# SamArgt/AudioSourceSep

Hardware: AMD Instinct MI355X
Metric: Glow fwd+logdet passes/sec on 64×64×1 mel tiles (K=32,L=3), 1→8 MI355X (higher is better)
Workload: dtype f16x3

## Files before the change

### audiosourcesep_amd/csrc/glowk_co.h

```cpp
#pragma once
#include "glowk_kernels.h"

constexpr int CO_PX = 128;
constexpr int CO_PSTR = 132;

template <int KIN, int MOUT, int NF, int MODE>
struct RingC {
  static constexpr int MODE7 = net_dir<MODE>;
  using S = RingS<KIN, MOUT, NF, MODE7, 2>;
  static constexpr bool FUSE = (MODE & NET_FUSE) != 0;
  static constexpr bool SAVE = MODE7 == NET_FWD_SAVE, BWD = MODE7 == NET_BWD;
  static constexpr bool MERGE = S::NMT <= 3;
  static constexpr bool M0LAST = S::NMT % 3 == 2;
  static constexpr bool STORE = (MODE & NET_STORE) != 0;
  static constexpr int MODEX = net_dir<MODE> | (MODE & NET_STORE);
  static constexpr int NFH = S::NFH, NRB = S::NRB, NMT = S::NMT, KS = S::KS;
  static constexpr int UNITP = S::MAINP / 2;
  static constexpr int UNIT4 = S::MAIN4 / 2;
  static constexpr int PPW = UNITP / 4;
  static constexpr int NG = NFH / 2;
  static constexpr int K1PW = (S::K1P + 3) / 4;
  static constexpr int EPN = BWD ? 0 : S::EPN;
  static constexpr int MASKN = BWD ? 2 * 4 * NF * 64 : 0;
  static constexpr size_t LDS_BYTES = (size_t)3 * UNIT4 * 16 + (size_t)2 * S::K14 * 16 + (size_t)EPN * 4 + (size_t)MASKN * 2 +
// ... 67 lines not shown
    acc2[o1][0] = __builtin_amdgcn_mfma_f32_16x16x32_f16(af[3], bh[0], acc2[o1][0], 0, 0, 0);
    acc2[o1][1] = __builtin_amdgcn_mfma_f32_16x16x32_f16(af[3], bh[1], acc2[o1][1], 0, 0, 0);
    if (MODE7 != NET_FWD2) {
      acc2[o0][0] = __builtin_amdgcn_mfma_f32_16x16x32_f16(af[0], bl[0], acc2[o0][0], 0, 0, 0);
      acc2[o0][1] = __builtin_amdgcn_mfma_f32_16x16x32_f16(af[0], bl[1], acc2[o0][1], 0, 0, 0);
      acc2[o1][0] = __builtin_amdgcn_mfma_f32_16x16x32_f16(af[2], bl[0], acc2[o1][0], 0, 0, 0);
      acc2[o1][1] = __builtin_amdgcn_mfma_f32_16x16x32_f16(af[2], bl[1], acc2[o1][1], 0, 0, 0);
    }
    acc2[o0][0] = __builtin_amdgcn_mfma_f32_16x16x32_f16(af[0], bh[0], acc2[o0][0], 0, 0, 0);
    acc2[o0][1] = __builtin_amdgcn_mfma_f32_16x16x32_f16(af[0], bh[1], acc2[o0][1], 0, 0, 0);
    acc2[o1][0] = __builtin_amdgcn_mfma_f32_16x16x32_f16(af[2], bh[0], acc2[o1][0], 0, 0, 0);
    acc2[o1][1] = __builtin_amdgcn_mfma_f32_16x16x32_f16(af[2], bh[1], acc2[o1][1], 0, 0, 0);
    __builtin_amdgcn_sched_barrier(0);
  }
}

template <int KIN, int MOUT, int NF, int MODE, int PASS, bool SOLO, int Z>
__device__ __forceinline__ void co_Z(const NetArgs& a, const H3Ctx& hc, const CoCtx& c, const float* epl, float* pl,
                                     f32x4 (&acc2)[(RingC<KIN, MOUT, NF, MODE>::NRB)][2], f32x4 (&acc3)[(RingC<KIN, MOUT, NF, MODE>::NMT)][2], h8 (&bh)[2],
                                     h8 (&bl)[2], const int (&q)[2], const bool (&qok)[2], int lane, int kq,
                                     f32x4 (&keep)[(RingC<KIN, MOUT, NF, MODE>::NMT)][2]) {
  using G = RingC<KIN, MOUT, NF, MODE>;
  constexpr int NFH = G::NFH, NMT = G::NMT, M3 = MOUT, MODE7 = G::MODE7;
  constexpr bool NEXT = !SOLO && PASS == 0;
  constexpr bool LAST = !SOLO && PASS == 1;
  if constexpr (NMT == 3) {
    if constexpr (Z == 0) stage4<G::UNITP, 70>(G::out_unit(c.img, PASS, 2), c.m1, c.w4, c.voff);
    if constexpr (Z == 1 && NEXT) stage4<G::UNITP, 71>(G::out_unit(c.img, PASS + 1, 0), c.d, c.w4, c.voff);
    if constexpr (Z == 2 && NEXT) stage4<G::UNITP, 72>(G::main_unit(c.img, PASS + 1, 0, 0), c.m0, c.w4, c.voff);
  } else if constexpr (NMT == 2) {
    if constexpr (Z == 0 && NEXT) stage4<G::UNITP, 75>(G::main_unit(c.img, PASS + 1, 0, 1), c.m1, c.w4, c.voff);
    if constexpr (Z == 1 && NEXT) stage4<G::UNITP, 76>(G::out_unit(c.img, PASS + 1, 0), c.d, c.w4, c.voff);
  } else {
    static_assert(NMT == 5, "conv3 units");
    if constexpr (Z == 0) stage4<G::UNITP, 80>(G::out_unit(c.img, PASS, 2), c.m1, c.w4, c.voff);
    if constexpr (Z == 1) stage4<G::UNITP, 81>(G::out_unit(c.img, PASS, 3), c.d, c.w4, c.voff);
    if constexpr (Z == 2) stage4<G::UNITP, 82>(G::out_unit(c.img, PASS, 4), c.m0, c.w4, c.voff);
    if constexpr (Z == 3 && NEXT) stage4<G::UNITP, 83>(G::main_unit(c.img, PASS + 1, 0, 1), c.m1, c.w4, c.voff);
    if constexpr (Z == 4 && NEXT) stage4<G::UNITP, 84>(G::out_unit(c.img, PASS + 1, 0), c.d, c.w4, c.voff);
  }
  const float4* slot = Z % 3 == 0 ? c.d : Z % 3 == 1 ? c.m0 : c.m1;
  const h8* buf = reinterpret_cast<const h8*>(slot) + lane;
  const float* pb = epl + NF * 32;
#pragma unroll
  for (int tp = 0; tp < NFH; ++tp) {
    const int t = Z * NFH + tp;
    const int fo = t / NMT, ml = t % NMT;
    if (ml == 0) {
      unsigned mask = 0, bits = 0;
      if (G::BWD) mask = hc.mkl[((size_t)(threadIdx.x >> 6) * NF + PASS * NFH + fo) * 64 + lane];
      if constexpr (G::STORE)
        bits = h3s_act_pair<MODE7, true>(acc2[2 * fo][0], acc2[2 * fo + 1][0], acc2[2 * fo][1], acc2[2 * fo + 1][1], a.sc2, mask, bh, bl,
                                         uniform_fptr(a.st2 + (size_t)(PASS * NFH + fo) * 32 * a.Q), ((unsigned)(4 * kq) * (unsigned)a.Q + (unsigned)q[0]) * 4u,
                                         (unsigned)a.Q * 4u);
      else {
#pragma unroll
        for (int hf = 0; hf < 2; ++hf) bits |= h3s_act<MODE7, false>(acc2[2 * fo][hf], acc2[2 * fo + 1][hf], a.sc2, mask >> (8 * hf), bh[hf], bl[hf]) << (8 * hf);
      }
      if (G::SAVE && hc.wok) a.mask2[(hc.wblk * NF + PASS * NFH + fo) * 64 + lane] = (unsigned short)bits;
    }
    if (fo == 0) {
#pragma unroll
      for (int r = 0; r < 4; ++r) { acc3[ml][0][r] = 0.0f; acc3[ml][1][r] = 0.0f; }
    }
    const h8 ah = buf[(tp * 2 + 0) * 64], al = buf[(tp * 2 + 1) * 64];
    acc3[ml][0] = mfma3s<MODE7 == NET_FWD2>(ah, al, bh[0], bl[0], acc3[ml][0]);
    acc3[ml][1] = mfma3s<MODE7 == NET_FWD2>(ah, al, bh[1], bl[1], acc3[ml][1]);
    if (fo == NFH - 1) {
#pragma unroll
      for (int hf = 0; hf < 2; ++hf)
#pragma unroll
        for (int r = 0; r < 4; ++r) {
          const int m = ml * 16 + 4 * kq + r;
          const float part = G::BWD ? acc3[ml][hf][r] * (a.sc3 * hc.ub[hf]) : PASS == 0 ? fmaf(acc3[ml][hf][r], a.sc3, pb[m]) : acc3[ml][hf][r] * a.sc3;
          if constexpr (NEXT && G::MERGE) { keep[ml][hf][r] = part; continue; }
          const float val = (LAST && G::MERGE) ? part + keep[ml][hf][r] : part;
          if constexpr (G::FUSE) {
            if (m < M3) pl[m * CO_PSTR + (int)(threadIdx.x >> 6) * 32 + 16 * hf + (lane & 15)] = val;
          } else {
            float* Pp = a.P + ((SOLO || !G::MERGE) ? (size_t)PASS * a.pstride : (size_t)0);
            if (m < M3 && qok[hf]) Pp[(size_t)m * a.Q + q[hf]] = val;
          }
        }
    }
  }
  constexpr bool ISSUED = NMT == 3 ? (Z == 0 || NEXT) : NMT == 2 ? (Z <= 1 && NEXT) : (Z <= 2 || NEXT);
  if constexpr (Z + 1 < NMT) {
    if constexpr (G::STORE) {
      constexpr int after = (ISSUED ? G::PPW : 0) + G::z_st(Z) + ((NMT == 3 && Z == 1) ? G::z_st(0) : 0);
      co_end<(after < 63 ? after : 63)>();
    } else if constexpr (G::SAVE) co_end<0>();
    else co_end<(ISSUED ? G::PPW : 0)>();
  } else co_bar();
}

template <int KIN, int MOUT, int NF, int MODE, int PASS, bool SOLO>
__device__ __forceinline__ void co_pass(const NetArgs& a, const H3Ctx& hc, const CoCtx& c, const float* epl, float* pl,
                                        const h8 (&xh)[(RingC<KIN, MOUT, NF, MODE>::KS)][2], const h8 (&xl)[(RingC<KIN, MOUT, NF, MODE>::KS)][2],
                                        const int (&q)[2], const bool (&qok)[2], int lane, int kq, f32x4 (&keep)[(RingC<KIN, MOUT, NF, MODE>::NMT)][2]) {
  using G = RingC<KIN, MOUT, NF, MODE>;
  using S = typename G::S;
  constexpr int NRB = G::NRB, NFH = G::NFH, MODE7 = G::MODE7;
  constexpr int f2base = PASS * NFH * 32;
  constexpr bool SECOND = !SOLO && PASS == 1;
  f32x4 acc2[NRB][2];
#pragma unroll
  for (int ob = 0; ob < NRB; ++ob)
#pragma unroll
    for (int r = 0; r < 4; ++r) {
      const float b = G::BWD ? 0.0f : epl[f2base + ob * 16 + 4 * kq + r];
      acc2[ob][0][r] = b;
      acc2[ob][1][r] = b;
    }
  const bool st = G::SAVE && PASS == 0 && hc.wok;
  constexpr int XST = PASS == 0 ? G::XST : 0;
  h8 bh[2], bl[2];
#pragma nounroll
  for (int i0 = 0; i0 < NF; i0 += 2) {
    if (i0 > 0 || (SECOND && !G::M0LAST)) stage4<G::UNITP, 73>(G::main_unit(c.img, PASS, i0, 1), c.m1, c.w4, c.voff);
    if constexpr (SECOND && G::M0LAST) {
      if (i0 == 0) stage4<G::UNITP, 77>(G::main_unit(c.img, PASS, 0, 0), c.m0, c.w4, c.voff);
    }
    h3s_X<KIN, MOUT, NF, G::MODEX, 2, 0, PASS, G::STORE>(a, hc, i0, xh, xl, lane, bh, bl);
    if (SECOND && G::M0LAST && i0 == 0) co_end<0>();
    else co_end_st<G::PPW + XST>(st);
    co_Y<NFH, MODE7, 0, 1, S::K1P>(c.m0, bh, bl, acc2, lane, hc.k1img + (size_t)((i0 + 2) % NF) * S::K14, hc.k1s0, c.w4, c.voff);
    co_end_st<G::K1PW + XST>(st);
    co_Y<NFH, MODE7, 1, 2, S::K1P>(c.m1, bh, bl, acc2, lane, G::main_unit(c.img, PASS, i0 + 1, 0), c.m0, c.w4, c.voff);
    co_bar();
    stage4<G::UNITP, 74>(G::main_unit(c.img, PASS, i0 + 1, 1), c.m1, c.w4, c.voff);
    h3s_X<KIN, MOUT, NF, G::MODEX, 2, 1, PASS, G::STORE>(a, hc, i0 + 1, xh, xl, lane, bh, bl);
    co_end_st<G::PPW + XST>(st);
    co_Y<NFH, MODE7, 0, 3, S::K1P>(c.m0, bh, bl, acc2, lane, hc.k1img + (size_t)((i0 + 3) % NF) * S::K14, hc.k1s1, c.w4, c.voff);
    co_end_st<G::K1PW + XST>(st);
    co_Y<NFH, MODE7, 1, 4, S::K1P>(c.m1, bh, bl, acc2, lane, i0 + 2 < NF ? G::main_unit(c.img, PASS, i0 + 2, 0) : G::out_unit(c.img, PASS, 1), c.m0,
                                   c.w4, c.voff);
    co_bar();
  }
  f32x4 acc3[G::NMT][2];
  co_Z<KIN, MOUT, NF, MODE, PASS, SOLO, 0>(a, hc, c, epl, pl, acc2, acc3, bh, bl, q, qok, lane, kq, keep);
  co_Z<KIN, MOUT, NF, MODE, PASS, SOLO, 1>(a, hc, c, epl, pl, acc2, acc3, bh, bl, q, qok, lane, kq, keep);
  if constexpr (G::NMT >= 3) co_Z<KIN, MOUT, NF, MODE, PASS, SOLO, 2>(a, hc, c, epl, pl, acc2, acc3, bh, bl, q, qok, lane, kq, keep);
  if constexpr (G::NMT >= 4) co_Z<KIN, MOUT, NF, MODE, PASS, SOLO, 3>(a, hc, c, epl, pl, acc2, acc3, bh, bl, q, qok, lane, kq, keep);
  if constexpr (G::NMT >= 5) co_Z<KIN, MOUT, NF, MODE, PASS, SOLO, 4>(a, hc, c, epl, pl, acc2, acc3, bh, bl, q, qok, lane, kq, keep);
}

struct CoCtxDB {
  float4 *s0, *s1, *s2, *s3;
  const float4* img;
  int w4;
  unsigned voff;
};

template <int NFH, int MODE7, int TAG, int K1P>
__device__ __forceinline__ void co_Ydb(const float4* sa, const float4* sb, const h8 (&bh)[2], const h8 (&bl)[2], f32x4 (&acc2)[2 * NFH][2], int lane,
                                       const float4* srca, float4* dsta, const float4* srcb, float4* dstb, const float4* k1src, float4* k1dst,
                                       int w4, unsigned voff) {
  const h8* bufa = reinterpret_cast<const h8*>(sa) + lane;
  const h8* bufb = reinterpret_cast<const h8*>(sb) + lane;
  const char* uba = uniform_ptr(srca);
  const char* ubb = uniform_ptr(srcb);
  constexpr int NG = NFH / 2;
  h8 A[2][4];
  auto load = [&](h8 (&d)[4], int g) {
    const h8* buf = g < NG ? bufa : bufb;
    const int gi = g % NG;
    d[0] = buf[((2 * gi) * 2 + 0) * 64];
    d[1] = buf[((2 * gi) * 2 + 1) * 64];
    d[2] = buf[((2 * gi + 1) * 2 + 0) * 64];
    d[3] = buf[((2 * gi + 1) * 2 + 1) * 64];
  };
  load(A[0], 0);
#pragma unroll
  for (int g = 0; g < 2 * NG; ++g) {
    const int gi = g % NG;
    const int o0 = (g / NG) * NFH + 2 * gi, o1 = o0 + 1;
    if (g + 1 < 2 * NG) load(A[(g + 1) & 1], g + 1);
    const int piece = gi * 4 + w4;
    if (g < NG) glds16(reinterpret_cast<const float4*>(uba + (size_t)piece * 1024 + voff), dsta + piece * 64);
    else glds16(reinterpret_cast<const float4*>(ubb + (size_t)piece * 1024 + voff), dstb + piece * 64);
    asm volatile("; dma site %0" ::"n"(TAG * 16 + g));
    if (g == 0) stage4<K1P, TAG * 16 + 15>(k1src, k1dst, w4, voff);
    __builtin_amdgcn_sched_barrier(0);
    const h8 (&af)[4] = A[g & 1];
    acc2[o0][0] = __builtin_amdgcn_mfma_f32_16x16x32_f16(af[1], bh[0], acc2[o0][0], 0, 0, 0);
    acc2[o0][1] = __builtin_amdgcn_mfma_f32_16x16x32_f16(af[1], bh[1], acc2[o0][1], 0, 0, 0);
    acc2[o1][0] = __builtin_amdgcn_mfma_f32_16x16x32_f16(af[3], bh[0], acc2[o1][0], 0, 0, 0);
    acc2[o1][1] = __builtin_amdgcn_mfma_f32_16x16x32_f16(af[3], bh[1], acc2[o1][1], 0, 0, 0);
    if (MODE7 != NET_FWD2) {
      acc2[o0][0] = __builtin_amdgcn_mfma_f32_16x16x32_f16(af[0], bl[0], acc2[o0][0], 0, 0, 0);
      acc2[o0][1] = __builtin_amdgcn_mfma_f32_16x16x32_f16(af[0], bl[1], acc2[o0][1], 0, 0, 0);
      acc2[o1][0] = __builtin_amdgcn_mfma_f32_16x16x32_f16(af[2], bl[0], acc2[o1][0], 0, 0, 0);
      acc2[o1][1] = __builtin_amdgcn_mfma_f32_16x16x32_f16(af[2], bl[1], acc2[o1][1], 0, 0, 0);
    }
    acc2[o0][0] = __builtin_amdgcn_mfma_f32_16x16x32_f16(af[0], bh[0], acc2[o0][0], 0, 0, 0);
    acc2[o0][1] = __builtin_amdgcn_mfma_f32_16x16x32_f16(af[0], bh[1], acc2[o0][1], 0, 0, 0);
    acc2[o1][0] = __builtin_amdgcn_mfma_f32_16x16x32_f16(af[2], bh[0], acc2[o1][0], 0, 0, 0);
    acc2[o1][1] = __builtin_amdgcn_mfma_f32_16x16x32_f16(af[2], bh[1], acc2[o1][1], 0, 0, 0);
    __builtin_amdgcn_sched_barrier(0);
  }
}

template <int KIN, int MOUT, int NF, int MODE, int PASS, int Z>
__device__ __forceinline__ void co_Zdb(const NetArgs& a, const CoCtxDB& c, const float* epl, f32x4 (&acc2)[(RingC<KIN, MOUT, NF, MODE>::NRB)][2],
                                       f32x4 (&acc3)[3][2], h8 (&bh)[2], h8 (&bl)[2], int lane, int kq, f32x4 (&keep)[3][2]) {
  using G = RingC<KIN, MOUT, NF, MODE>;
  constexpr int NFH = G::NFH, NMT = G::NMT, M3 = MOUT, MODE7 = G::MODE7;
  static_assert(NMT == 3 && G::MERGE && G::FUSE, "the double-buffered ring: three conv3 units, merged passes, fused coupling");
  constexpr bool NEXT = PASS == 0;
  if constexpr (Z == 0) stage4<G::UNITP, 90>(G::out_unit(c.img, PASS, 2), c.s2, c.w4, c.voff);
  if constexpr (Z == 1 && NEXT) stage4<G::UNITP, 91>(G::main_unit(c.img, PASS + 1, 0, 0), c.s0, c.w4, c.voff);
  if constexpr (Z == 2 && NEXT) stage4<G::UNITP, 92>(G::main_unit(c.img, PASS + 1, 0, 1), c.s1, c.w4, c.voff);
  const float4* slot = Z == 0 ? c.s0 : Z == 1 ? c.s1 : c.s2;
  const h8* buf = reinterpret_cast<const h8*>(slot) + lane;
  const float* pb = epl + NF * 32;
#pragma unroll
  for (int tp = 0; tp < NFH; ++tp) {
    const int t = Z * NFH + tp;
    const int fo = t / NMT, ml = t % NMT;
    if (ml == 0) {
#pragma unroll
      for (int hf = 0; hf < 2; ++hf) h3s_act<MODE7, false>(acc2[2 * fo][hf], acc2[2 * fo + 1][hf], a.sc2, 0u, bh[hf], bl[hf]);
    }
    if (fo == 0) {
#pragma unroll
      for (int r = 0; r < 4; ++r) { acc3[ml][0][r] = 0.0f; acc3[ml][1][r] = 0.0f; }
    }
    const h8 ah = buf[(tp * 2 + 0) * 64], al = buf[(tp * 2 + 1) * 64];
    acc3[ml][0] = mfma3s<MODE7 == NET_FWD2>(ah, al, bh[0], bl[0], acc3[ml][0]);
    acc3[ml][1] = mfma3s<MODE7 == NET_FWD2>(ah, al, bh[1], bl[1], acc3[ml][1]);
    if (fo == NFH - 1) {
      float* pt = reinterpret_cast<float*>(ml == 0 ? c.s0 : ml == 1 ? c.s1 : c.s3);
#pragma unroll
      for (int hf = 0; hf < 2; ++hf)
#pragma unroll
        for (int r = 0; r < 4; ++r) {
          const int m = ml * 16 + 4 * kq + r;
          const float part = PASS == 0 ? fmaf(acc3[ml][hf][r], a.sc3, pb[m]) : acc3[ml][hf][r] * a.sc3;
          if constexpr (NEXT) { keep[ml][hf][r] = part; continue; }
          const float val = part + keep[ml][hf][r];
          if (m < M3) pt[(4 * kq + r) * CO_PSTR + (int)(threadIdx.x >> 6) * 32 + 16 * hf + (lane & 15)] = val;
        }
    }
  }
  if constexpr (Z == 0) co_bar();
  if constexpr (Z == 1) co_end<(NEXT ? G::PPW : 0)>();
  if constexpr (Z == 2 && NEXT) co_bar();
}

template <int KIN, int MOUT, int NF, int MODE, int PASS>
__device__ __forceinline__ void co_pass_db(const NetArgs& a, const H3Ctx& hc, const CoCtxDB& c, const float* epl,
                                           const h8 (&xh)[(RingC<KIN, MOUT, NF, MODE>::KS)][2], const h8 (&xl)[(RingC<KIN, MOUT, NF, MODE>::KS)][2],
                                           int lane, int kq, f32x4 (&keep)[3][2]) {
  using G = RingC<KIN, MOUT, NF, MODE>;
  using S = typename G::S;
  constexpr int NRB = G::NRB, NFH = G::NFH, MODE7 = G::MODE7;
  constexpr int f2base = PASS * NFH * 32;
  f32x4 acc2[NRB][2];
#pragma unroll
  for (int ob = 0; ob < NRB; ++ob)
#pragma unroll
    for (int r = 0; r < 4; ++r) {
      const float b = epl[f2base + ob * 16 + 4 * kq + r];
      acc2[ob][0][r] = b;
      acc2[ob][1][r] = b;
    }
  h8 bh[2], bl[2];
#pragma nounroll
  for (int i0 = 0; i0 < NF; i0 += 2) {
    h3s_X<KIN, MOUT, NF, G::MODEX, 2, 0, PASS, false>(a, hc, i0, xh, xl, lane, bh, bl);
    co_end<0>();
    co_Ydb<NFH, MODE7, 1, S::K1P>(c.s0, c.s1, bh, bl, acc2, lane, G::main_unit(c.img, PASS, i0 + 1, 0), c.s2, G::main_unit(c.img, PASS, i0 + 1, 1), c.s3,
                                  hc.k1img + (size_t)((i0 + 2) % NF) * S::K14, hc.k1s0, c.w4, c.voff);
    h3s_X<KIN, MOUT, NF, G::MODEX, 2, 1, PASS, false>(a, hc, i0 + 1, xh, xl, lane, bh, bl);
    co_end<0>();
    const bool more = i0 + 2 < NF;
    co_Ydb<NFH, MODE7, 2, S::K1P>(c.s2, c.s3, bh, bl, acc2, lane, more ? G::main_unit(c.img, PASS, i0 + 2, 0) : G::out_unit(c.img, PASS, 0), c.s0,
                                  more ? G::main_unit(c.img, PASS, i0 + 2, 1) : G::out_unit(c.img, PASS, 1), c.s1,
                                  hc.k1img + (size_t)((i0 + 3) % NF) * S::K14, hc.k1s1, c.w4, c.voff);
  }
  co_end<0>();
  f32x4 acc3[3][2];
  co_Zdb<KIN, MOUT, NF, MODE, PASS, 0>(a, c, epl, acc2, acc3, bh, bl, lane, kq, keep);
  co_Zdb<KIN, MOUT, NF, MODE, PASS, 1>(a, c, epl, acc2, acc3, bh, bl, lane, kq, keep);
  co_Zdb<KIN, MOUT, NF, MODE, PASS, 2>(a, c, epl, acc2, acc3, bh, bl, lane, kq, keep);
}

template <int KIN, int MOUT, int NF, int MODE, bool SPLIT, bool RING3 = false>
__global__ __launch_bounds__(256, 2) void k_net_h3c(NetArgs a) {
  using G = RingC<KIN, MOUT, NF, MODE>;
  using S = typename G::S;
  constexpr int KS = G::KS;
  constexpr int SGN = G::BWD ? -1 : 1;
  static_assert(G::FITS, "shape");
  static_assert(!(G::FUSE && SPLIT), "the fused coupling needs both passes in one workgroup");
  constexpr bool DB = G::DB && !SPLIT && !RING3;
  static_assert(!RING3 || G::DB, "RING3 names the three-slot form of an instance that has both");
  static_assert(!DB || 2 * G::LDS_BYTES_DB <= 160 * 1024, "two workgroups per CU");

  const int tid = threadIdx.x;
  CoCtx c;
  CoCtxDB cd;
  if constexpr (DB) {
    __shared__ __attribute__((aligned(1024))) float4 slotS0[G::DBSLOT4];
    __shared__ __attribute__((aligned(1024))) float4 slotS1[G::DBSLOT4];
    __shared__ __attribute__((aligned(1024))) float4 slotS2[G::DBSLOT4];
    __shared__ __attribute__((aligned(1024))) float4 slotS3[G::DBSLOT4];
    cd.s0 = slotS0; cd.s1 = slotS1; cd.s2 = slotS2; cd.s3 = slotS3;
  } else {
    __shared__ __attribute__((aligned(1024))) float4 slotM0[G::UNIT4];
    __shared__ __attribute__((aligned(1024))) float4 slotM1[G::UNIT4];
    __shared__ __attribute__((aligned(1024))) float4 slotD[G::UNIT4];
    c.m0 = slotM0; c.m1 = slotM1; c.d = slotD;
  }
  __shared__ __attribute__((aligned(1024))) float4 k1slot0[S::K14];
  __shared__ __attribute__((aligned(1024))) float4 k1slot1[S::K14];
  float* epl = nullptr;
  if constexpr (!G::BWD) { __shared__ float epl_arr[S::EPN]; epl = epl_arr; }
  unsigned short* mkl = nullptr;
  if constexpr (G::BWD) { __shared__ __attribute__((aligned(1024))) unsigned short mkl_arr[G::MASKN]; mkl = mkl_arr; }
  float* plds = nullptr;
  float4* vstash = nullptr;
  if constexpr (G::FUSE && !DB) { __shared__ float plds_arr[36 * CO_PSTR]; plds = plds_arr; }
  if constexpr (G::FUSE) { __shared__ float4 vstash_arr[CO_PX]; vstash = vstash_arr; }
  const int lane = tid & 63;
  const int wave = __builtin_amdgcn_readfirstlane(tid >> 6);
  const int n16 = lane & 15;
  const int kq = lane >> 4;
  const int qbase = ((int)blockIdx.x * 4 + wave) * 32;
  const int q[2] = {G::STORE ? qbase + 2 * n16 : qbase + n16, G::STORE ? qbase + 2 * n16 + 1 : qbase + 16 + n16};
  const bool qok[2] = {q[0] < a.Q, q[1] < a.Q};
  const int pass0 = SPLIT ? (int)blockIdx.y : 0;

  H3Ctx hc;
  hc.sA = hc.sB = hc.sD = nullptr; hc.k1s0 = k1slot0; hc.k1s1 = k1slot1;
  hc.k1img = a.RSp; hc.img = a.RSp; hc.mkl = mkl; hc.mk2off = 4 * NF * 64; hc.pl = plds;
  hc.wblk = (size_t)blockIdx.x * 4 + wave;
  hc.wok = (long)hc.wblk * 32 < a.Q;
  hc.w4 = wave; hc.voff = (unsigned)lane * 16u; hc.ub[0] = hc.ub[1] = 1.0f;
  c.img = a.RSp; c.w4 = wave; c.voff = (unsigned)lane * 16u;
  cd.img = a.RSp; cd.w4 = wave; cd.voff = (unsigned)lane * 16u;

  if constexpr (DB) {
    stage4<G::UNITP, 58>(G::main_unit(cd.img, 0, 0, 0), cd.s0, c.w4, c.voff);
    stage4<G::UNITP, 59>(G::main_unit(cd.img, 0, 0, 1), cd.s1, c.w4, c.voff);
  } else {
    stage4<G::UNITP, 60>(G::main_unit(c.img, pass0, 0, 0), c.m0, c.w4, c.voff);
    stage4<G::UNITP, 61>(G::main_unit(c.img, pass0, 0, 1), c.m1, c.w4, c.voff);
    stage4<G::UNITP, 62>(G::out_unit(c.img, pass0, 0), c.d, c.w4, c.voff);
  }
  stage4<S::K1P, 63>(hc.k1img, k1slot0, c.w4, c.voff);
  stage4<S::K1P, 64>(hc.k1img + S::K14, k1slot1, c.w4, c.voff);
  if constexpr (G::BWD) {
    stage4<NF / 2, 65>(reinterpret_cast<const float4*>(a.mask1 + (size_t)blockIdx.x * 4 * NF * 64), reinterpret_cast<float4*>(mkl), c.w4, c.voff);
    stage4<NF / 2, 66>(reinterpret_cast<const float4*>(a.mask2 + (size_t)blockIdx.x * 4 * NF * 64), reinterpret_cast<float4*>(mkl + 4 * NF * 64), c.w4, c.voff);
  }

  h8 xh[KS][2], xl[KS][2];
  float xmax = 0.0f;
  {
    const int hw = a.h * a.w;
#pragma unroll
    for (int hf = 0; hf < 2; ++hf) {
      const int qq = qok[hf] ? q[hf] : 0;
      const int rem = qq % hw;
      const int i = rem / a.w, j0 = rem % a.w;
      const float* base = a.vin + (long)qq * a.in_stride + a.in_off;
      if constexpr (G::BWD) {
        float v[KS][8];
        float pm = 0.0f;
#pragma unroll
        for (int s = 0; s < KS; ++s) {
          gather8<KIN, false, SGN>(base, i, j0, a.h, a.w, a.in_stride, qok[hf], 32 * s + 8 * kq, v[s]);
          pm = range8(pm, v[s]);
        }
        pm = nan_max(pm, __shfl_xor(pm, 16, 64));
        pm = nan_max(pm, __shfl_xor(pm, 32, 64));
        xmax = nan_max(xmax, pm);
        const float fac = G::STORE ? 1.0f : pixel_norm(pm, a.bnorm, hc.ub[hf]);
#pragma unroll
        for (int s = 0; s < KS; ++s) {
#pragma unroll
          for (int j = 0; j < 8; ++j) v[s][j] *= fac;
          split8(v[s], xh[s][hf], xl[s][hf]);
        }
      } else if constexpr (S::STK) {
        xmax = gather_stacked<KIN, SGN, G::MODE7 == NET_FWD2, KS, S::KSX>(base, i, j0, a.h, a.w, a.in_stride, qok[hf], kq, xh, xl, hf, xmax);
      } else {
#pragma unroll
        for (int s = 0; s < KS; ++s) {
          float v[8];
          gather8<KIN, true, SGN>(base, i, j0, a.h, a.w, a.in_stride, qok[hf], 32 * s + 8 * kq, v);
          xmax = range8(xmax, v);
          split8(v, xh[s][hf], xl[s][hf]);
        }
      }
    }
  }
  if constexpr (G::FUSE) {
    if (tid < CO_PX) {
      const int qv = (int)blockIdx.x * CO_PX + tid;
      vstash[tid] = qv < a.Q ? *reinterpret_cast<const float4*>(a.vin + (size_t)qv * 4) : float4{0.f, 0.f, 0.f, 0.f};
    }
  }
  if constexpr (!G::BWD)
    for (int i = tid; i < S::EPN; i += 256) epl[i] = a.eph[i];
  if (((G::BWD && !G::STORE) ? !(xmax <= 3.0e38f) : !(xmax <= a.xlim)) && a.flag) *a.flag = 1;
  if (a.xmax_out) range_probe(a.xmax_out, xmax);
  asm volatile("s_waitcnt vmcnt(0)" ::: "memory");
  __syncthreads();

  f32x4 keep[G::NMT][2];
  if constexpr (DB) {
    co_pass_db<KIN, MOUT, NF, MODE, 0>(a, hc, cd, epl, xh, xl, lane, kq, keep);
    co_pass_db<KIN, MOUT, NF, MODE, 1>(a, hc, cd, epl, xh, xl, lane, kq, keep);
    __syncthreads();
    fused_couple<CO_PX, CO_PSTR>(a, reinterpret_cast<const float*>(cd.s0), reinterpret_cast<const float*>(cd.s1), reinterpret_cast<const float*>(cd.s3), vstash, tid);
  } else if constexpr (SPLIT) {
    if (pass0 == 0) co_pass<KIN, MOUT, NF, MODE, 0, true>(a, hc, c, epl, plds, xh, xl, q, qok, lane, kq, keep);
    else co_pass<KIN, MOUT, NF, MODE, 1, true>(a, hc, c, epl, plds, xh, xl, q, qok, lane, kq, keep);
  } else {
    co_pass<KIN, MOUT, NF, MODE, 0, false>(a, hc, c, epl, plds, xh, xl, q, qok, lane, kq, keep);
    co_pass<KIN, MOUT, NF, MODE, 1, false>(a, hc, c, epl, plds, xh, xl, q, qok, lane, kq, keep);
  }
  if constexpr (G::FUSE && !DB) {
    __syncthreads();
    fused_couple<CO_PX, CO_PSTR>(a, plds, vstash, tid);
  }
}
```

### audiosourcesep_amd/csrc/glowk_kernels.h

```cpp
#pragma once
#include "glowk_act_scale.h"

#include <hip/hip_runtime.h>
#include <utility>
#include <stdint.h>

typedef float f32x16 __attribute__((ext_vector_type(16)));

#define GLOWK_GPTR(p) ((const __attribute__((address_space(1))) void*)(p))
#define GLOWK_LPTR(p) ((__attribute__((address_space(3))) void*)(p))

__device__ __forceinline__ int mfma_row(int r, int hh) { return (r & 3) + 8 * (r >> 2) + 4 * hh; }

struct NetArgs {
  const float* vin;
  int in_stride, in_off;
  int Q, h, w;
  const float* K1p;
  const float* ep;
  const float4* R0p;
  unsigned short* mask1;
  unsigned short* mask2;
  float* P;
  size_t pstride;
// ... 911 lines not shown
  static constexpr int IMG_NCH = (IMGH * NMT + 2 * IMGH - 1) / (2 * IMGH);
  static constexpr int IMG_PASS4 = (NF + IMG_NCH) * IMG_MAIN4;
  static constexpr int SUBS = NP / 2;
  __device__ static const float4* main_chunk(const float4* img, int pass, int ch) {
    return img + K1TOT4 + (size_t)(pass / SUBS) * IMG_PASS4 + (size_t)ch * IMG_MAIN4 + (size_t)(pass % SUBS) * MAIN4;
  }
  __device__ static const float4* out_chunk(const float4* img, int pass, int s) {
    const int sub = pass % SUBS, t4 = s * TPC;
    const int gi = t4 / GT;
    const int t2 = IMGH * 6 * gi + sub * NFH * grp_n(gi) + (t4 - GT * gi);
    return img + K1TOT4 + (size_t)(pass / SUBS) * IMG_PASS4 + (size_t)NF * IMG_MAIN4 + (size_t)t2 * 128;
  }
  static constexpr int tile_fo(int t) { return (t - GT * (t / GT)) / grp_n(t / GT); }
  static constexpr int tile_mt(int t) { return 6 * (t / GT) + (t - GT * (t / GT)) % grp_n(t / GT); }
  static constexpr bool MERGE = PXH == 2 && NP == 2 && NGRP == 1 && NMT <= 3 &&
                                (net_dir<MODE> == NET_FWD || net_dir<MODE> == NET_FWD2 || (net_dir<MODE> == NET_BWD && NMT <= 2) || (net_dir<MODE> == NET_FWD_SAVE && FUSE));
};

template <bool TWO = false>
__device__ __forceinline__ f32x4 mfma3s(const h8& ahi, const h8& alo, const h8& bhi, const h8& blo, f32x4 acc) {
  acc = __builtin_amdgcn_mfma_f32_16x16x32_f16(alo, bhi, acc, 0, 0, 0);
  if (!TWO) acc = __builtin_amdgcn_mfma_f32_16x16x32_f16(ahi, blo, acc, 0, 0, 0);
  acc = __builtin_amdgcn_mfma_f32_16x16x32_f16(ahi, bhi, acc, 0, 0, 0);
  return acc;
}

template <int MODE>
__device__ __forceinline__ unsigned h3s_act_vals(const f32x4& r0, const f32x4& r1, float sc, unsigned mask8, float (&v)[8]) {
  unsigned bits = 0;
#pragma unroll
  for (int j = 0; j < 8; j += 2) {
    const f32x2 a2 = j < 4 ? f32x2{r0[j], r0[j + 1]} : f32x2{r1[j - 4], r1[j - 3]};
    const f32x2 t2 = a2 * f32x2{sc, sc};
    const float t[2] = {t2.x, t2.y}, av[2] = {a2.x, a2.y};
#pragma unroll
    for (int e = 0; e < 2; ++e) {
      if (MODE == NET_BWD) v[j + e] = __int_as_float(__float_as_int(t[e]) & __builtin_amdgcn_sbfe((int)mask8, j + e, 1));
      else {
        v[j + e] = fmaxf(t[e], 0.0f);
        if (MODE == NET_FWD_SAVE) bits |= (av[e] > 0.0f ? 1u : 0u) << (j + e);
      }
    }
  }
  return bits;
}
template <int MODE, bool ST = false>
__device__ __forceinline__ unsigned h3s_act(const f32x4& r0, const f32x4& r1, float sc, unsigned mask8, h8& bh, h8& bl, bool do_st = false,
                                            float* st_blk = nullptr, unsigned st_lane = 0, unsigned st_row = 0) {
  float v[8];
  const unsigned bits = h3s_act_vals<MODE>(r0, r1, sc, mask8, v);
  if constexpr (ST) {
    if (do_st) {
      const unsigned long long st_base = reinterpret_cast<unsigned long long>(st_blk);
#pragma unroll
      for (int j = 0; j < 8; ++j) {
        const unsigned off = st_lane + (unsigned)((j >> 2) * 16 + (j & 3)) * st_row;
        asm volatile("global_store_dword %0, %1, %2" GLOWK_ST_MOD ::"v"(off), "v"(v[j]), "s"(st_base) : "memory");
      }
    }
  }
  if (MODE == NET_FWD2) {
#pragma unroll
    for (int j = 0; j < 8; ++j) { bh[j] = (_Float16)v[j]; bl[j] = (_Float16)0.0f; }
  } else split8(v, bh, bl);
  return bits;
}
template <int MODE, bool ST>
__device__ __forceinline__ unsigned h3s_act_pair(const f32x4& r00, const f32x4& r10, const f32x4& r01, const f32x4& r11, float sc, unsigned mask16,
                                                 h8 (&bh)[2], h8 (&bl)[2], float* st_blk, unsigned st_lane, unsigned st_row) {
  float v0[8], v1[8];
  unsigned bits = h3s_act_vals<MODE>(r00, r10, sc, mask16, v0);
  bits |= h3s_act_vals<MODE>(r01, r11, sc, mask16 >> 8, v1) << 8;
  if constexpr (ST) {
    const unsigned long long st_base = reinterpret_cast<unsigned long long>(st_blk);
#pragma unroll
    for (int j = 0; j < 8; ++j) {
      const unsigned off = st_lane + (unsigned)((j >> 2) * 16 + (j & 3)) * st_row;
      const f32x2 pr = {v0[j], v1[j]};
      asm volatile("global_store_dwordx2 %0, %1, %2" GLOWK_ST_MOD ::"v"(off), "v"(pr), "s"(st_base) : "memory");
    }
  }
  split8(v0, bh[0], bl[0]);
  split8(v1, bh[1], bl[1]);
  return bits;
}

template <int KIN, int MOUT, int NF, int MODE, int NP, int KP, int PASS, bool PAIR = false>
__device__ __forceinline__ void h3s_X(const NetArgs& a, const H3Ctx& c, int fi, const h8 (&xh)[(RingS<KIN, MOUT, NF, MODE, NP>::KS)][2],
                                      const h8 (&xl)[(RingS<KIN, MOUT, NF, MODE, NP>::KS)][2], int lane, h8 (&bh)[2], h8 (&bl)[2]) {
  using G = RingS<KIN, MOUT, NF, MODE, NP>;
  unsigned mask = 0;
  if (net_dir<MODE> == NET_BWD) mask = c.mkl[c.mk2off + ((size_t)(threadIdx.x >> 6) * NF + fi) * 64 + lane];
  f32x4 h1[2][2];
#pragma unroll
  for (int i = 0; i < 4; ++i)
#pragma unroll
    for (int r = 0; r < 4; ++r) h1[i >> 1][i & 1][r] = 0.0f;
  const h8* k1 = reinterpret_cast<const h8*>(KP ? c.k1s1 : c.k1s0) + lane;
  if constexpr (G::STK) {
    static_assert(G::KSX <= 6, "operand reads in flight");
    h8 kf[G::KSX * 2];
#pragma unroll
    for (int i = 0; i < G::KSX * 2; ++i) kf[i] = k1[i * 64];
    __builtin_amdgcn_sched_barrier(0);
#pragma unroll
    for (int s = 0; s < G::KSX; ++s)
#pragma unroll
      for (int rb = 0; rb < 2; ++rb)
#pragma unroll
        for (int hf = 0; hf < G::PXH; ++hf)
          h1[rb][hf] = __builtin_amdgcn_mfma_f32_16x16x32_f16(kf[s * 2 + rb], x_frag(xh, xl, s, hf), h1[rb][hf], 0, 0, 0);
  } else if constexpr (G::KS <= 3) {
    h8 kf[G::K1P];
#pragma unroll
    for (int i = 0; i < G::K1P; ++i) kf[i] = k1[i * 64];
    __builtin_amdgcn_sched_barrier(0);
#pragma unroll
    for (int s = 0; s < G::KS; ++s)
#pragma unroll
      for (int rb = 0; rb < 2; ++rb)
#pragma unroll
        for (int hf = 0; hf < G::PXH; ++hf)
          h1[rb][hf] = mfma3s<net_dir<MODE> == NET_FWD2>(kf[(s * 2 + rb) * 2 + 0], kf[(s * 2 + rb) * 2 + 1], xh[s][hf], xl[s][hf], h1[rb][hf]);
  } else {
#pragma unroll
    for (int s = 0; s < G::KS; ++s)
#pragma unroll
      for (int rb = 0; rb < 2; ++rb) {
        const h8 ah = k1[((s * 2 + rb) * 2 + 0) * 64], al = k1[((s * 2 + rb) * 2 + 1) * 64];
#pragma unroll
        for (int hf = 0; hf < G::PXH; ++hf) h1[rb][hf] = mfma3s<net_dir<MODE> == NET_FWD2>(ah, al, xh[s][hf], xl[s][hf], h1[rb][hf]);
      }
  }
  unsigned bits = 0;
  if constexpr (PAIR) {
    static_assert(G::PXH == 2, "pairs: two pixel halves per wave");
    const int stq = (int)c.wblk * 32 + 2 * (lane & 15);
    if constexpr ((MODE & NET_STORE) && PASS == 0)
      bits = h3s_act_pair<net_dir<MODE>, true>(h1[0][0], h1[1][0], h1[0][1], h1[1][1], a.sc1, mask, bh, bl, uniform_fptr(a.st1 + (size_t)fi * 32 * a.Q),
                                            ((unsigned)(4 * (lane >> 4)) * (unsigned)a.Q + (unsigned)stq) * 4u, (unsigned)a.Q * 4u);
    else bits = h3s_act_pair<net_dir<MODE>, false>(h1[0][0], h1[1][0], h1[0][1], h1[1][1], a.sc1, mask, bh, bl, nullptr, 0u, 0u);
  } else {
#pragma unroll
    for (int hf = 0; hf < G::PXH; ++hf) {
      const int stq = (int)c.wblk * (16 * G::PXH) + 16 * hf + (lane & 15);
      bits |= h3s_act<net_dir<MODE>, (MODE & NET_STORE) != 0>(h1[0][hf], h1[1][hf], a.sc1, mask >> (8 * hf), bh[hf], bl[hf], (MODE & NET_STORE) && PASS == 0 && stq < a.Q,
                                                   (MODE & NET_STORE) ? uniform_fptr(a.st1 + (size_t)fi * 32 * a.Q) : nullptr,
                                                   ((unsigned)(4 * (lane >> 4)) * (unsigned)a.Q + (unsigned)stq) * 4u, (unsigned)a.Q * 4u) << (8 * hf);
    }
  }
  if (net_dir<MODE> == NET_FWD_SAVE && PASS == 0 && c.wok) a.mask1[(c.wblk * NF + fi) * 64 + lane] = (unsigned short)bits;
}

template <int KIN, int MOUT, int NF, int MODE, int NP, int TAG>
__device__ __forceinline__ void h3s_Y(const float4* slot, const h8 (&bh)[2], const h8 (&bl)[2], f32x4 (&acc2)[(RingS<KIN, MOUT, NF, MODE, NP>::NRB)][2],
                                      int lane, int g, bool main_ok, const float4* main_src, float4* main_dst, const float4* k1_src,
                                      float4* k1_dst, int w4, unsigned voff) {
  using G = RingS<KIN, MOUT, NF, MODE, NP>;
  const h8* buf = reinterpret_cast<const h8*>(slot) + lane;
  const char* mb = uniform_ptr(main_src);
  constexpr int NG = G::NRB / 2;
  constexpr int PPG = G::MAINP / 4 / NG;
  h8 A[2][4];
  auto load = [&](h8 (&d)[4], int gi) {
    d[0] = buf[((2 * gi) * 2 + 0) * 64];
    d[1] = buf[((2 * gi) * 2 + 1) * 64];
    d[2] = buf[((2 * gi + 1) * 2 + 0) * 64];
    d[3] = buf[((2 * gi + 1) * 2 + 1) * 64];
  };
  load(A[0], 0);
#pragma unroll
  for (int gi = 0; gi < NG; ++gi) {
    const int o0 = 2 * gi, o1 = 2 * gi + 1;
    if (gi + 1 < NG) load(A[(gi + 1) & 1], gi + 1);
    if (!g) {
      if (main_ok) {
#pragma unroll
        for (int e = 0; e < PPG; ++e) {
          const int piece = (gi * PPG + e) * 4 + w4;
          glds16(reinterpret_cast<const float4*>(mb + (size_t)piece * 1024 + voff), main_dst + piece * 64);
        }
      }
      asm volatile("; dma site %0" ::"n"(TAG * 16 + gi));
    } else if (gi == 0) {
      stage4<G::K1P, TAG * 16 + 15>(k1_src, k1_dst, w4, voff);
    }
    __builtin_amdgcn_sched_barrier(0);
    const h8 (&af)[4] = A[gi & 1];
    acc2[o0][0] = __builtin_amdgcn_mfma_f32_16x16x32_f16(af[1], bh[0], acc2[o0][0], 0, 0, 0);
    if constexpr (G::PXH == 2) acc2[o0][1] = __builtin_amdgcn_mfma_f32_16x16x32_f16(af[1], bh[1], acc2[o0][1], 0, 0, 0);
    acc2[o1][0] = __builtin_amdgcn_mfma_f32_16x16x32_f16(af[3], bh[0], acc2[o1][0], 0, 0, 0);
    if constexpr (G::PXH == 2) acc2[o1][1] = __builtin_amdgcn_mfma_f32_16x16x32_f16(af[3], bh[1], acc2[o1][1], 0, 0, 0);
    if (net_dir<MODE> != NET_FWD2) {
      acc2[o0][0] = __builtin_amdgcn_mfma_f32_16x16x32_f16(af[0], bl[0], acc2[o0][0], 0, 0, 0);
      if constexpr (G::PXH == 2) acc2[o0][1] = __builtin_amdgcn_mfma_f32_16x16x32_f16(af[0], bl[1], acc2[o0][1], 0, 0, 0);
      acc2[o1][0] = __builtin_amdgcn_mfma_f32_16x16x32_f16(af[2], bl[0], acc2[o1][0], 0, 0, 0);
      if constexpr (G::PXH == 2) acc2[o1][1] = __builtin_amdgcn_mfma_f32_16x16x32_f16(af[2], bl[1], acc2[o1][1], 0, 0, 0);
    }
    acc2[o0][0] = __builtin_amdgcn_mfma_f32_16x16x32_f16(af[0], bh[0], acc2[o0][0], 0, 0, 0);
    if constexpr (G::PXH == 2) acc2[o0][1] = __builtin_amdgcn_mfma_f32_16x16x32_f16(af[0], bh[1], acc2[o0][1], 0, 0, 0);
    acc2[o1][0] = __builtin_amdgcn_mfma_f32_16x16x32_f16(af[2], bh[0], acc2[o1][0], 0, 0, 0);
    if constexpr (G::PXH == 2) acc2[o1][1] = __builtin_amdgcn_mfma_f32_16x16x32_f16(af[2], bh[1], acc2[o1][1], 0, 0, 0);
    __builtin_amdgcn_sched_barrier(0);
  }
}

template <int KIN, int MOUT, int NF, int MODE, int NP, int P0, int PASS, bool SOLO, int Z>
__device__ __forceinline__ void h3s_Z(const NetArgs& a, const H3Ctx& c, const float* epl, f32x4 (&acc2)[(RingS<KIN, MOUT, NF, MODE, NP>::NRB)][2],
                                      f32x4 (&acc3)[(RingS<KIN, MOUT, NF, MODE, NP>::G0N)][2], h8 (&bh)[2], h8 (&bl)[2], int g, const int (&q)[2],
                                      const bool (&qok)[2], int lane, int kq, f32x4 (&keep)[(RingS<KIN, MOUT, NF, MODE, NP>::G0N)][2]) {
  using G = RingS<KIN, MOUT, NF, MODE, NP>;
  constexpr int NFH = G::NFH, M3 = G::M3, TPC = G::TPC;
  constexpr bool MERGE = G::MERGE && !SOLO;
  constexpr int S = Z >> 1;
  constexpr int P0N = (G::NCH + 1 + P0) & 1;
  if (!g) {
    constexpr int SN = Z == 1 ? 2 : (Z >= 5 && (Z & 1)) ? (Z + 1) / 2 : 0;
    if constexpr (SN >= 2 && SN < G::NCH)
      stage4<G::MAINP, 16 + Z>(G::out_chunk(c.img, PASS, SN), ((NF + SN - 1 + P0) & 1) ? c.sB : c.sA, c.w4, c.voff);
    if constexpr (PASS + 1 < NP && !SOLO && Z == 2 * G::NCH - 1) {
      stage4<G::MAINP, 48>(G::main_chunk(c.img, PASS + 1, 0), P0N ? c.sB : c.sA, c.w4, c.voff);
      if constexpr (G::NCH >= 2) stage4<G::MAINP, 49>(G::out_chunk(c.img, PASS + 1, 0), c.sD, c.w4, c.voff);
    }
  }
  const float4* slot = S == 0 ? c.sD : (((NF + S - 1 + P0) & 1) ? c.sB : c.sA);
  const h8* buf = reinterpret_cast<const h8*>(slot) + lane;
  float* Pp = a.P + (MERGE ? (size_t)0 : (size_t)PASS * a.pstride);
  const float* pb = epl + NF * 32;
#pragma unroll
  for (int i = 0; i < TPC / 2; ++i) {
    const int tp = (Z & 1) * (TPC / 2) + i;
    const int t = S * TPC + tp;
    if (t < G::NT) {
      const int fo = G::tile_fo(t), mt = G::tile_mt(t);
      const int ml = mt % 6;
      if (ml == 0) {
        unsigned mask = 0, bits = 0;
        if (net_dir<MODE> == NET_BWD) mask = c.mkl[((size_t)(threadIdx.x >> 6) * NF + PASS * NFH + fo) * 64 + lane];
#pragma unroll
        for (int hf = 0; hf < G::PXH; ++hf)
          bits |= h3s_act<net_dir<MODE>, (MODE & NET_STORE) != 0>(acc2[2 * fo][hf], acc2[2 * fo + 1][hf], a.sc2, mask >> (8 * hf), bh[hf], bl[hf], (MODE & NET_STORE) && qok[hf],
                                                       (MODE & NET_STORE) ? uniform_fptr(a.st2 + (size_t)(PASS * NFH + fo) * 32 * a.Q) : nullptr,
                                                       ((unsigned)(4 * kq) * (unsigned)a.Q + (unsigned)q[hf]) * 4u, (unsigned)a.Q * 4u) << (8 * hf);
        if (net_dir<MODE> == NET_FWD_SAVE && t < NFH * G::G0N && c.wok) a.mask2[(c.wblk * NF + PASS * NFH + fo) * 64 + lane] = (unsigned short)bits;
      }
      if (fo == 0) {
#pragma unroll
        for (int r = 0; r < 4; ++r) { acc3[ml][0][r] = 0.0f; acc3[ml][1][r] = 0.0f; }
      }
      const h8 ah = buf[(tp * 2 + 0) * 64], al = buf[(tp * 2 + 1) * 64];
      acc3[ml][0] = mfma3s<net_dir<MODE> == NET_FWD2>(ah, al, bh[0], bl[0], acc3[ml][0]);
      if constexpr (G::PXH == 2) acc3[ml][1] = mfma3s<net_dir<MODE> == NET_FWD2>(ah, al, bh[1], bl[1], acc3[ml][1]);
      if (fo == NFH - 1) {
#pragma unroll
        for (int hf = 0; hf < G::PXH; ++hf)
#pragma unroll
          for (int r = 0; r < 4; ++r) {
            const int m = mt * 16 + 4 * kq + r;
            const float val = net_dir<MODE> == NET_BWD ? acc3[ml][hf][r] * (a.sc3 * c.ub[hf])
                              : PASS == 0 ? fmaf(acc3[ml][hf][r], a.sc3, pb[m]) : acc3[ml][hf][r] * a.sc3;
            if (MERGE && PASS == 0) { keep[ml][hf][r] = val; continue; }
            if constexpr (G::FUSE) {
              if (m < M3) c.pl[m * FUSE_PSTR + (int)(threadIdx.x >> 6) * 32 + 16 * hf + (lane & 15)] = val + keep[ml][hf][r];
              continue;
            }
            if (m < M3 && qok[hf]) Pp[(size_t)m * a.Q + q[hf]] = MERGE ? val + keep[ml][hf][r] : val;
          }
      }
    }
  }
  h3_wait_barrier();
}

template <int KIN, int MOUT, int NF, int MODE, int NP, int P0, int PASS, bool SOLO, int... Z>
__device__ __forceinline__ void h3s_tail(const NetArgs& a, const H3Ctx& c, const float* epl, f32x4 (&acc2)[(RingS<KIN, MOUT, NF, MODE, NP>::NRB)][2],
                                         f32x4 (&acc3)[(RingS<KIN, MOUT, NF, MODE, NP>::G0N)][2], h8 (&bh)[2], h8 (&bl)[2], int g, const int (&q)[2],
                                         const bool (&qok)[2], int lane, int kq, f32x4 (&keep)[(RingS<KIN, MOUT, NF, MODE, NP>::G0N)][2],
                                         std::integer_sequence<int, Z...>) {
  (h3s_Z<KIN, MOUT, NF, MODE, NP, P0, PASS, SOLO, Z>(a, c, epl, acc2, acc3, bh, bl, g, q, qok, lane, kq, keep), ...);
}

template <int KIN, int MOUT, int NF, int MODE, int NP, int P0, int PASS, bool SOLO>
__device__ __forceinline__ void h3s_pass(const NetArgs& a, const H3Ctx& c, const float* epl, const h8 (&xh)[(RingS<KIN, MOUT, NF, MODE, NP>::KS)][2],
                                         const h8 (&xl)[(RingS<KIN, MOUT, NF, MODE, NP>::KS)][2], int g, const int (&q)[2], const bool (&qok)[2], int lane, int kq,
                                         f32x4 (&keep)[(RingS<KIN, MOUT, NF, MODE, NP>::G0N)][2]) {
  using G = RingS<KIN, MOUT, NF, MODE, NP>;
  constexpr int NRB = G::NRB;
  constexpr int f2base = PASS * G::NFH * 32;
  f32x4 acc2[NRB][2];
#pragma unroll
  for (int ob = 0; ob < NRB; ++ob)
#pragma unroll
    for (int r = 0; r < 4; ++r) {
      const float b = net_dir<MODE> == NET_BWD ? 0.0f : epl[f2base + ob * 16 + 4 * kq + r];
      acc2[ob][0][r] = b;
      acc2[ob][1][r] = b;
    }
  h8 bh[2], bl[2];
#pragma nounroll
  for (int i0 = 0; i0 < NF; i0 += 2) {
    h3s_X<KIN, MOUT, NF, MODE, NP, 0, PASS>(a, c, i0, xh, xl, lane, bh, bl);
    h3_x_end<MODE, PASS, 8 * G::PXH>(c);
    if (PASS >= 1 && !SOLO && G::NCH == 1 && i0 == 0 && !g)
      stage4<G::MAINP, 50>(G::out_chunk(c.img, PASS, 0), c.sD, c.w4, c.voff);
    h3s_Y<KIN, MOUT, NF, MODE, NP, 1>(P0 ? c.sB : c.sA, bh, bl, acc2, lane, g, true, G::main_chunk(c.img, PASS, i0 + 1), P0 ? c.sA : c.sB,
                         c.k1img + (size_t)((i0 + 2) % NF) * G::K14, c.k1s0, c.w4, c.voff);
// ... 232 lines not shown
```

Before: 16740.

## Software-pipeline conv1 weight and first A-fragment loads across the double-buffered ring

After: 16920 (median of 6 runs). +1.1%, better.

```diff
diff --git a/audiosourcesep_amd/csrc/glowk_co.h b/audiosourcesep_amd/csrc/glowk_co.h
--- a/audiosourcesep_amd/csrc/glowk_co.h
+++ b/audiosourcesep_amd/csrc/glowk_co.h
@@ -243,16 +243,16 @@
   unsigned voff;
 };
 
-template <int NFH, int MODE7, int TAG, int K1P>
+template <int NFH, int MODE7, int TAG, int K1P, int NKF>
 __device__ __forceinline__ void co_Ydb(const float4* sa, const float4* sb, const h8 (&bh)[2], const h8 (&bl)[2], f32x4 (&acc2)[2 * NFH][2], int lane,
-                                       const float4* srca, float4* dsta, const float4* srcb, float4* dstb, const float4* k1src, float4* k1dst,
-                                       int w4, unsigned voff) {
+                                       h8 (&A)[2][4], h8 (&kf)[NKF], const float4* kslot, const float4* srca, float4* dsta, const float4* srcb,
+                                       float4* dstb, const float4* k1src, float4* k1dst, int w4, unsigned voff) {
   const h8* bufa = reinterpret_cast<const h8*>(sa) + lane;
   const h8* bufb = reinterpret_cast<const h8*>(sb) + lane;
+  const h8* kbuf = reinterpret_cast<const h8*>(kslot) + lane;
   const char* uba = uniform_ptr(srca);
   const char* ubb = uniform_ptr(srcb);
   constexpr int NG = NFH / 2;
-  h8 A[2][4];
   auto load = [&](h8 (&d)[4], int g) {
     const h8* buf = g < NG ? bufa : bufb;
     const int gi = g % NG;
@@ -261,23 +261,30 @@
     d[2] = buf[((2 * gi + 1) * 2 + 0) * 64];
     d[3] = buf[((2 * gi + 1) * 2 + 1) * 64];
   };
-  load(A[0], 0);
 #pragma unroll
   for (int g = 0; g < 2 * NG; ++g) {
     const int gi = g % NG;
     const int o0 = (g / NG) * NFH + 2 * gi, o1 = o0 + 1;
-    if (g + 1 < 2 * NG) load(A[(g + 1) & 1], g + 1);
-    const int piece = gi * 4 + w4;
-    if (g < NG) glds16(reinterpret_cast<const float4*>(uba + (size_t)piece * 1024 + voff), dsta + piece * 64);
-    else glds16(reinterpret_cast<const float4*>(ubb + (size_t)piece * 1024 + voff), dstb + piece * 64);
-    asm volatile("; dma site %0" ::"n"(TAG * 16 + g));
-    if (g == 0) stage4<K1P, TAG * 16 + 15>(k1src, k1dst, w4, voff);
-    __builtin_amdgcn_sched_barrier(0);
     const h8 (&af)[4] = A[g & 1];
     acc2[o0][0] = __builtin_amdgcn_mfma_f32_16x16x32_f16(af[1], bh[0], acc2[o0][0], 0, 0, 0);
     acc2[o0][1] = __builtin_amdgcn_mfma_f32_16x16x32_f16(af[1], bh[1], acc2[o0][1], 0, 0, 0);
     acc2[o1][0] = __builtin_amdgcn_mfma_f32_16x16x32_f16(af[3], bh[0], acc2[o1][0], 0, 0, 0);
     acc2[o1][1] = __builtin_amdgcn_mfma_f32_16x16x32_f16(af[3], bh[1], acc2[o1][1], 0, 0, 0);
+    __builtin_amdgcn_sched_barrier(0);
+    if (g + 1 < 2 * NG) load(A[(g + 1) & 1], g + 1);
+    else {
+#pragma unroll
+      for (int i = 0; i < NKF; ++i) kf[i] = kbuf[i * 64];
+    }
+    if (g < NG) {
+      const int piece = g * 4 + w4;
+      glds16(reinterpret_cast<const float4*>(uba + (size_t)piece * 1024 + voff), dsta + piece * 64);
+      asm volatile("; dma site %0" ::"n"(TAG * 16 + g));
+      glds16(reinterpret_cast<const float4*>(ubb + (size_t)piece * 1024 + voff), dstb + piece * 64);
+      asm volatile("; dma site %0" ::"n"(TAG * 16 + NG + g));
+    }
+    if (g == 0) stage4<K1P, TAG * 16 + 15>(k1src, k1dst, w4, voff);
+    __builtin_amdgcn_sched_barrier(0);
     if (MODE7 != NET_FWD2) {
       acc2[o0][0] = __builtin_amdgcn_mfma_f32_16x16x32_f16(af[0], bl[0], acc2[o0][0], 0, 0, 0);
       acc2[o0][1] = __builtin_amdgcn_mfma_f32_16x16x32_f16(af[0], bl[1], acc2[o0][1], 0, 0, 0);
@@ -290,6 +297,25 @@
     acc2[o1][1] = __builtin_amdgcn_mfma_f32_16x16x32_f16(af[2], bh[1], acc2[o1][1], 0, 0, 0);
     __builtin_amdgcn_sched_barrier(0);
   }
+}
+
+template <int KIN, int MOUT, int NF, int MODE>
+__device__ __forceinline__ void co_Xdb(const NetArgs& a, const h8 (&xh)[(RingC<KIN, MOUT, NF, MODE>::KS)][2], const h8 (&xl)[(RingC<KIN, MOUT, NF, MODE>::KS)][2],
+                                       int lane, const h8 (&kf)[(RingC<KIN, MOUT, NF, MODE>::S::KSX * 2)], const float4* sa, h8 (&A0)[4], h8 (&bh)[2],
+                                       h8 (&bl)[2]) {
+  using G = RingC<KIN, MOUT, NF, MODE>;
+  f32x4 h1[2][2];
+  h3s_X_mma<typename G::S>(kf, xh, xl, h1);
+#pragma unroll
+  for (int i = 0; i < 4; ++i) asm volatile("" : "+v"(h1[i >> 1][i & 1]));
+  __builtin_amdgcn_sched_barrier(0);
+  co_end<0>();
+  const h8* buf = reinterpret_cast<const h8*>(sa) + lane;
+#pragma unroll
+  for (int j = 0; j < 4; ++j) A0[j] = buf[j * 64];
+  __builtin_amdgcn_sched_barrier(0);
+  h3s_X_act<G::MODE7>(h1, a.sc1, bh, bl);
+  __builtin_amdgcn_sched_barrier(0);
 }
 
 template <int KIN, int MOUT, int NF, int MODE, int PASS, int Z>
@@ -357,18 +383,21 @@
       acc2[ob][1][r] = b;
     }
   h8 bh[2], bl[2];
+  constexpr int NKF = S::KSX * 2;
+  h8 A[2][4];
+  h8 kf[NKF];
+  h3s_X_load<S, 0>(hc, lane, kf);
+  __builtin_amdgcn_sched_barrier(0);
 #pragma nounroll
   for (int i0 = 0; i0 < NF; i0 += 2) {
-    h3s_X<KIN, MOUT, NF, G::MODEX, 2, 0, PASS, false>(a, hc, i0, xh, xl, lane, bh, bl);
-    co_end<0>();
-    co_Ydb<NFH, MODE7, 1, S::K1P>(c.s0, c.s1, bh, bl, acc2, lane, G::main_unit(c.img, PASS, i0 + 1, 0), c.s2, G::main_unit(c.img, PASS, i0 + 1, 1), c.s3,
-                                  hc.k1img + (size_t)((i0 + 2) % NF) * S::K14, hc.k1s0, c.w4, c.voff);
-    h3s_X<KIN, MOUT, NF, G::MODEX, 2, 1, PASS, false>(a, hc, i0 + 1, xh, xl, lane, bh, bl);
-    co_end<0>();
+    co_Xdb<KIN, MOUT, NF, MODE>(a, xh, xl, lane, kf, c.s0, A[0], bh, bl);
+    co_Ydb<NFH, MODE7, 1, S::K1P, NKF>(c.s0, c.s1, bh, bl, acc2, lane, A, kf, hc.k1s1, G::main_unit(c.img, PASS, i0 + 1, 0), c.s2,
+                                       G::main_unit(c.img, PASS, i0 + 1, 1), c.s3, hc.k1img + (size_t)((i0 + 2) % NF) * S::K14, hc.k1s0, c.w4, c.voff);
+    co_Xdb<KIN, MOUT, NF, MODE>(a, xh, xl, lane, kf, c.s2, A[0], bh, bl);
     const bool more = i0 + 2 < NF;
-    co_Ydb<NFH, MODE7, 2, S::K1P>(c.s2, c.s3, bh, bl, acc2, lane, more ? G::main_unit(c.img, PASS, i0 + 2, 0) : G::out_unit(c.img, PASS, 0), c.s0,
-                                  more ? G::main_unit(c.img, PASS, i0 + 2, 1) : G::out_unit(c.img, PASS, 1), c.s1,
-                                  hc.k1img + (size_t)((i0 + 3) % NF) * S::K14, hc.k1s1, c.w4, c.voff);
+    co_Ydb<NFH, MODE7, 2, S::K1P, NKF>(c.s2, c.s3, bh, bl, acc2, lane, A, kf, hc.k1s0, more ? G::main_unit(c.img, PASS, i0 + 2, 0) : G::out_unit(c.img, PASS, 0),
+                                       c.s0, more ? G::main_unit(c.img, PASS, i0 + 2, 1) : G::out_unit(c.img, PASS, 1), c.s1,
+                                       hc.k1img + (size_t)((i0 + 3) % NF) * S::K14, hc.k1s1, c.w4, c.voff);
   }
   co_end<0>();
   f32x4 acc3[3][2];
diff --git a/audiosourcesep_amd/csrc/glowk_kernels.h b/audiosourcesep_amd/csrc/glowk_kernels.h
--- a/audiosourcesep_amd/csrc/glowk_kernels.h
+++ b/audiosourcesep_amd/csrc/glowk_kernels.h
@@ -1087,6 +1087,35 @@
   if (net_dir<MODE> == NET_FWD_SAVE && PASS == 0 && c.wok) a.mask1[(c.wblk * NF + fi) * 64 + lane] = (unsigned short)bits;
 }
 
+template <class G, int KP>
+__device__ __forceinline__ void h3s_X_load(const H3Ctx& c, int lane, h8 (&kf)[G::KSX * 2]) {
+  static_assert(G::STK && G::KSX <= 6, "stacked conv1; operand reads in flight");
+  const h8* k1 = reinterpret_cast<const h8*>(KP ? c.k1s1 : c.k1s0) + lane;
+#pragma unroll
+  for (int i = 0; i < G::KSX * 2; ++i) kf[i] = k1[i * 64];
+}
+template <class G>
+__device__ __forceinline__ void h3s_X_mma(const h8 (&kf)[G::KSX * 2], const h8 (&xh)[G::KS][2], const h8 (&xl)[G::KS][2], f32x4 (&h1)[2][2]) {
+  static_assert(G::STK && G::PXH == 2, "stacked conv1, two pixel halves per wave");
+#pragma unroll
+  for (int i = 0; i < 4; ++i)
+#pragma unroll
+    for (int r = 0; r < 4; ++r) h1[i >> 1][i & 1][r] = 0.0f;
+#pragma unroll
+  for (int s = 0; s < G::KSX; ++s)
+#pragma unroll
+    for (int rb = 0; rb < 2; ++rb)
+#pragma unroll
+      for (int hf = 0; hf < 2; ++hf)
+        h1[rb][hf] = __builtin_amdgcn_mfma_f32_16x16x32_f16(kf[s * 2 + rb], x_frag(xh, xl, s, hf), h1[rb][hf], 0, 0, 0);
+}
+template <int MODE7>
+__device__ __forceinline__ void h3s_X_act(const f32x4 (&h1)[2][2], float sc1, h8 (&bh)[2], h8 (&bl)[2]) {
+  static_assert(MODE7 == NET_FWD || MODE7 == NET_FWD2, "plain forward network");
+#pragma unroll
+  for (int hf = 0; hf < 2; ++hf) h3s_act<MODE7, false>(h1[0][hf], h1[1][hf], sc1, 0u, bh[hf], bl[hf]);
+}
+
 template <int KIN, int MOUT, int NF, int MODE, int NP, int TAG>
 __device__ __forceinline__ void h3s_Y(const float4* slot, const h8 (&bh)[2], const h8 (&bl)[2], f32x4 (&acc2)[(RingS<KIN, MOUT, NF, MODE, NP>::NRB)][2],
                                       int lane, int g, bool main_ok, const float4* main_src, float4* main_dst, const float4* k1_src,
```
